# silvadirceu/acoss-1

Measured on AMD Instinct MI355X. Metric: song-pairs/sec (CSM+Qmax) on 12-d HPCP, ~2000 frames/track; MAP parity, higher is better.
Workload: dtype f32; 1 GPU; covers80-shaped synthetic HPCP (hard corpus), Serra09 CRP+Qmax, all unordered pairs; tracks=164, frames_per_track=2000, m=9, tau=1, oti=True, parallelism=pair-matrix row stripes dp1

## Files before the change

### acoss-1_amd/csrc/crp_lines.hpp

```cpp
#pragma once
#include "common.hpp"

__device__ int acoss_writelane(int value, int lane, int old) __asm("llvm.amdgcn.writelane.i32");

namespace acoss {

constexpr unsigned kNone = 0x7fffu;

__device__ __forceinline__ unsigned pk_min_u16(unsigned a, unsigned b) {
  typedef unsigned short u16x2 __attribute__((ext_vector_type(2)));
  return __builtin_bit_cast(unsigned, __builtin_elementwise_min(__builtin_bit_cast(u16x2, a), __builtin_bit_cast(u16x2, b)));
}
__device__ __forceinline__ unsigned pk_max_u16(unsigned a, unsigned b) {
  typedef unsigned short u16x2 __attribute__((ext_vector_type(2)));
  return __builtin_bit_cast(unsigned, __builtin_elementwise_max(__builtin_bit_cast(u16x2, a), __builtin_bit_cast(u16x2, b)));
}
__device__ __forceinline__ unsigned pk_add_u16(unsigned a, unsigned b) {
  typedef unsigned short u16x2 __attribute__((ext_vector_type(2)));
  return __builtin_bit_cast(unsigned, __builtin_bit_cast(u16x2, a) + __builtin_bit_cast(u16x2, b));
}
__device__ __forceinline__ unsigned pk_subsat_u16(unsigned a, unsigned b) {
  typedef unsigned short u16x2 __attribute__((ext_vector_type(2)));
  return __builtin_bit_cast(unsigned, __builtin_elementwise_sub_sat(__builtin_bit_cast(u16x2, a), __builtin_bit_cast(u16x2, b)));
}
// ... 132 lines not shown
#pragma unroll
    for (int h = 0; h < NP; ++h) ne = gather_flags(ne, (pv[h] ^ PP) + 0x7fff7fffu, h);
    return ~ne;
  }
  __device__ __forceinline__ uint32_t le8(unsigned x) const {
    const unsigned X4 = (x - base8 + 0x80u) * 0x01010101u;
    uint32_t le8 = 0;
#pragma unroll
    for (int h = 0; h < NP / 2; ++h) le8 = gather_flags8(le8, X4 - w8[h], h);
    return le8;
  }
  __device__ __forceinline__ uint32_t le16(unsigned x) const {
    const unsigned X2 = (x + 0x8000u) * 0x10001u;
    uint32_t le = 0;
#pragma unroll
    for (int h = 0; h < NP; ++h) le = gather_flags(le, X2 - pv[h], h);
    return le;
  }
  __device__ __forceinline__ void min_max_lane(unsigned* a_io, unsigned* b_io) const {
    unsigned a = *a_io, b = *b_io;
#pragma unroll
    for (int h = 0; h < NP; ++h) {
      a = pk_min_u16(a, pv[h]);
      b = pk_max_u16(b, pk_add_u16(pv[h], 0x00010001u) & 0x7fff7fffu);
    }
    *a_io = a;
    *b_io = b;
  }
  static __device__ __forceinline__ void min_max_wave(unsigned a, unsigned b, unsigned* mn, unsigned* mx) {
    a = min(a & 0xffffu, a >> 16);
    b = max(b & 0xffffu, b >> 16);
    *mn = wave_min_u32(a);
    const unsigned m = wave_max_u32(b);
    *mx = m ? m - 1 : 0u;
  }
  __device__ __forceinline__ void min_max(unsigned* mn, unsigned* mx) const {
    unsigned a = 0xffffffffu, b = 0u;
    min_max_lane(&a, &b);
    min_max_wave(a, b, mn, mx);
  }
  __device__ __forceinline__ unsigned min_greater_lane(unsigned x) const { return swar_min_greater(pv, x); }
  __device__ __forceinline__ unsigned min_greater(unsigned x) const { return wave_min_u32(min_greater_lane(x)); }
  static constexpr bool kHist = true;
  __device__ __forceinline__ bool hist_rank(unsigned hint, int rho, unsigned* hist, unsigned* P, int* le,
                                            int* less, unsigned* hbase) const {
    if constexpr (WIN) {
      *hbase = base8;
      const bool exact0 = base8 == 0u;
      hist_fill_w8(w8, hist);
      return hist_place(hist, rho, base8, 0, exact0, P, le, less);
    } else {
      const unsigned base = hint > 64u ? hint - 64u : 0u;
      *hbase = base;
      hist_clear(hist);
      const HistAddr HA(hist);
      const unsigned below = base > 0u ? cnt16(base - 1u) : 0u;
#pragma unroll
      for (int h = 0; h < NP; ++h) {
#pragma unroll
        for (int half = 0; half < 2; ++half) {
          const unsigned c = (half ? (pv[h] >> 16) : (pv[h] & 0xffffu)) - base;
          hist_add(hist, HA, c, c < 128u);
        }
      }
      return hist_place(hist, rho, base, wave_sum((int)below), true, P, le, less);
    }
  }
};

template <int KPL>
struct Line : Codes<KPL / 2, true> {
  static_assert(KPL == 32, "split word order assumes 32 elements per lane");
  static constexpr int kHalves = 1;
  __device__ __forceinline__ int ebase() const {
    int e = (threadIdx.x & 63) * KPL;
    asm volatile("" : "+v"(e));
    return e;
  }
  __device__ __forceinline__ int elem(int eb, int b) const { return eb + b; }
  static __device__ __forceinline__ int lane_of(int e) { return e / KPL; }
  static __device__ __forceinline__ int bit_of(int e) { return e % KPL; }
  __device__ __forceinline__ unsigned sample() const { return this->pv[0] & 0xffffu; }
  template <bool STORED_SPLIT>
  __device__ __forceinline__ void load_lanes(const uint16_t* col0, size_t lane_stride, int n) {
    const int lane = threadIdx.x & 63;
    const int base = lane * KPL;
    const uint16_t* src = col0 + (base < n ? (size_t)lane * lane_stride : (size_t)0);
    this->no_window();
    unsigned w[KPL / 2];
#pragma unroll
    for (int q = 0; q < KPL / 8; ++q) {
      const uint4 v = reinterpret_cast<const uint4*>(src)[q];
      w[4 * q + 0] = v.x;
      w[4 * q + 1] = v.y;
      w[4 * q + 2] = v.z;
      w[4 * q + 3] = v.w;
    }
    if (STORED_SPLIT) {
#pragma unroll
      for (int h = 0; h < KPL / 2; ++h) this->pv[h] = w[h];
    } else {
#pragma unroll
      for (int h = 0; h < KPL / 2; ++h)
        this->pv[h] = __builtin_amdgcn_perm(w[8 + (h >> 1)], w[h >> 1], (h & 1) ? 0x07060302u : 0x05040100u);
    }
    if (base >= n) {
#pragma unroll
      for (int h = 0; h < KPL / 2; ++h) this->pv[h] = kNone * 0x10001u;
    }
  }
  __device__ __forceinline__ uint32_t eq_mask(unsigned P) const {
    if (this->eq_in_win(P)) return this->eq8(P);
    return this->eq16(P);
  }
  __device__ __forceinline__ uint32_t le_mask(unsigned x) const {
    if (this->in_win(x)) return this->le8(x);
    return this->le16(x);
  }
};

template <int KQ>
struct LineS : Codes<KQ / 2, KQ == 16> {
  static_assert(KQ == 8 || KQ == 16, "short lines: 8 or 16 elements per lane");
  static constexpr bool kWin = KQ == 16;
  static constexpr int kHalves = 1;
  static constexpr uint32_t kMaskAll = ((1u << (KQ / 2)) - 1u) * 0x10001u;
  static constexpr uint32_t kWinLo = ((1u << (KQ / 4)) - 1u) * 0x10001u;
  static __device__ __forceinline__ uint32_t wmask(uint32_t m) {
    return (m & kWinLo) | ((m >> (8 - KQ / 4)) & (kWinLo << (KQ / 4)));
  }
  static __device__ __forceinline__ int q_of_bit(int b) { return b < 16 ? b : b - 16 + KQ / 2; }
  static __device__ __forceinline__ int bit_of_q(int q) { return q < KQ / 2 ? q : q - KQ / 2 + 16; }
  __device__ __forceinline__ int ebase() const {
    int e = threadIdx.x & 63;
    asm volatile("" : "+v"(e));
    return e;
  }
  __device__ __forceinline__ int elem(int eb, int b) const { return eb + 64 * q_of_bit(b); }
  static __device__ __forceinline__ int lane_of(int e) { return e & 63; }
  static __device__ __forceinline__ int bit_of(int e) { return bit_of_q(e >> 6); }
  __device__ __forceinline__ unsigned sample() const {
    const int lane = threadIdx.x & 63;
    unsigned t[KQ / 2];
#pragma unroll
    for (int k = 0; k < KQ / 2; ++k) t[k] = this->pv[k];
#pragma unroll
    for (int bit = 1, n = KQ / 2; n > 1; bit <<= 1, n >>= 1) {
      const bool sel = (lane & bit) != 0;
#pragma unroll
      for (int k = 0; k < n / 2; ++k) t[k] = sel ? t[2 * k + 1] : t[2 * k];
    }
    return (lane & (KQ / 2)) ? (t[0] >> 16) : (t[0] & 0xffffu);
  }
  template <class AT>
  __device__ __forceinline__ void load(AT addr, int n) {
    const int lane = threadIdx.x & 63;
    this->no_window();
    unsigned v[KQ];
#pragma unroll
    for (int q = 0; q < KQ; ++q) v[q] = *addr(min(lane + 64 * q, n - 1));
#pragma unroll
    for (int q = 0; q < KQ; ++q) v[q] = lane + 64 * q < n ? v[q] : kNone;
#pragma unroll
    for (int h = 0; h < KQ / 2; ++h) this->pv[h] = v[h] | (v[h + KQ / 2] << 16);
  }
  __device__ __forceinline__ uint32_t eq_mask(unsigned P) const {
    if constexpr (kWin) {
      if (this->in_win(P) && (P > this->base8 || this->base8 == 0u)) return wmask(this->eq8(P));
    }
    return this->eq16(P) & kMaskAll;
  }
  __device__ __forceinline__ uint32_t le_mask(unsigned x) const {
    if constexpr (kWin) {
      if (this->in_win(x)) return wmask(this->le8(x));
    }
    return this->le16(x);
  }
};

template <int KQ>
__device__ __forceinline__ uint32_t lane_words(uint32_t mask) {
  uint32_t out = 0;
#pragma unroll
  for (int q = 0; q < KQ; ++q) {
    const unsigned long long bal = __ballot((mask >> LineS<KQ>::bit_of_q(q)) & 1u);
    out = (uint32_t)acoss_writelane((int)(uint32_t)bal, 2 * q, (int)out);
    out = (uint32_t)acoss_writelane((int)(uint32_t)(bal >> 32), 2 * q + 1, (int)out);
  }
  return out;
}

struct Line2 {
  Line<32> A, B;
  static constexpr int kHalves = 2;
  static constexpr bool kHist = false;
  __device__ __forceinline__ int ebase() const { return A.ebase(); }
  __device__ __forceinline__ int elem(int eb, int b) const { return b < 32 ? eb + b : 2048 + eb + (b - 32); }
  static __device__ __forceinline__ int lane_of(int e) { return e < 2048 ? (e >> 5) : 64 + ((e - 2048) >> 5); }
  static __device__ __forceinline__ int bit_of(int e) { return e & 31; }
  __device__ __forceinline__ unsigned sample() const {
    const unsigned a = A.sample(), b = B.sample();
    return (threadIdx.x & 1) ? b : a;
  }
  __device__ __forceinline__ void build_window(unsigned c) {
    A.build_window(c);
    B.build_window(c);
  }
  __device__ __forceinline__ int count_le(unsigned x) const {
    if (A.in_win(x)) return wave_sum((int)(A.cnt8(x) + B.cnt8(x)));
    return wave_sum((int)(A.cnt16(x) + B.cnt16(x)));
  }
  __device__ __forceinline__ uint64_t eq_mask(unsigned P) const {
    if (A.eq_in_win(P)) return (uint64_t)A.eq8(P) | ((uint64_t)B.eq8(P) << 32);
    return (uint64_t)A.eq16(P) | ((uint64_t)B.eq16(P) << 32);
  }
  __device__ __forceinline__ uint64_t le_mask(unsigned x) const {
    if (A.in_win(x)) return (uint64_t)A.le8(x) | ((uint64_t)B.le8(x) << 32);
    return (uint64_t)A.le16(x) | ((uint64_t)B.le16(x) << 32);
  }
  __device__ __forceinline__ void min_max(unsigned* mn, unsigned* mx) const {
    unsigned a = 0xffffffffu, b = 0u;
    A.min_max_lane(&a, &b);
    B.min_max_lane(&a, &b);
    Line<32>::min_max_wave(a, b, mn, mx);
  }
  __device__ __forceinline__ unsigned min_greater(unsigned x) const {
    return wave_min_u32(min(A.min_greater_lane(x), B.min_greater_lane(x)));
  }
};

}
```

### acoss-1_amd/csrc/crp_split.hip

```cpp
#include <cstdlib>
#include <cstring>
#include <type_traits>

#include "crp_internal.hpp"
#include "crp_lines.hpp"

namespace acoss {

namespace {

constexpr int kMS = 9;


struct PairView {
  const float* X;
  const float* X2;
  const float* Yr;
  int nq, nr, tau;
  const float* NXq;
  const float* NXr;
  int Mp, Np;
};

__device__ __forceinline__ PairView pair_view(const CrpBatch& B, int p) {
// ... 177 lines not shown
      }
    }
    typedef __attribute__((address_space(1))) char gchar;
    typedef uint32_t u32x4 __attribute__((ext_vector_type(4)));
    typedef __attribute__((address_space(1))) u32x4 gu4;
    u32x4* tq = reinterpret_cast<u32x4*>(tile);
    const int cc = lane - (kMS - 1);
    if (jb + kSysCols > V.Np) {
#pragma unroll
      for (int h = 0; h < 16; ++h) hw[h] = col < V.Np ? hw[h] : kNone * 0x10001u;
    }
    if (cc >= 0) {
      uint16_t* tc = tile + cc;
#pragma unroll
      for (int h = 0; h < 16; ++h) {
        tc[h * kSysCols] = (uint16_t)hw[h];
        tc[(h + 16) * kSysCols] = (uint16_t)(hw[h] >> 16);
      }
    }
    __builtin_amdgcn_wave_barrier();
    u32x4 pr[4], pq[4];
#pragma unroll
    for (int k = 0; k < 4; ++k) pr[k] = tq[min(lane + 64 * k, kTilePieces - 1)];
#pragma unroll
    for (int k = 0; k < 4; ++k) asm volatile("" : "+v"(pr[k].x), "+v"(pr[k].y), "+v"(pr[k].z), "+v"(pr[k].w));
#pragma unroll
    for (int k = 0; k < 4; ++k) {
      const int t = lane + 64 * k;
      const int row = t / 7;
      const int c = jb + 8 * (t - 7 * row);
      if (t < kTilePieces && c < V.Np && (!PARTIAL || row < rows))
        *(gu4*)((gchar*)(gu16*)Hr + (unsigned)(row * ldr + c) * 2u) = pr[k];
    }
    __builtin_amdgcn_wave_barrier();
    if (cc >= 0) {
      const int f = (cc >> 1) & 3;
#pragma unroll
      for (int q = 0; q < 4; ++q) tq[cc * 4 + (q ^ f)] = u32x4{hw[4 * q], hw[4 * q + 1], hw[4 * q + 2], hw[4 * q + 3]};
    }
    __builtin_amdgcn_wave_barrier();
#pragma unroll
    for (int k = 0; k < 4; ++k) {
      const int t = min(lane + 64 * k, kTilePieces - 1), c = t >> 2;
      pq[k] = tq[c * 4 + ((t & 3) ^ ((c >> 1) & 3))];
    }
#pragma unroll
    for (int k = 0; k < 4; ++k) asm volatile("" : "+v"(pq[k].x), "+v"(pq[k].y), "+v"(pq[k].z), "+v"(pq[k].w));
    __builtin_amdgcn_wave_barrier();
    gu16* hcb = (gu16*)(Hc + ((size_t)strip * ldc + jb) * kSR);
#pragma unroll
    for (int k = 0; k < 4; ++k) {
      const int t = lane + 64 * k;
      if (t < kTilePieces && jb + (t >> 2) < V.Np)
        __builtin_nontemporal_store(pq[k], (gu4*)((gchar*)hcb + (unsigned)t * 16u));
    }
  }
  __syncthreads();
  const int padw = (int)((V.Np + 31) & ~31) - V.Np;
  for (int e = threadIdx.x; e < kSR * 32; e += kThreads) {
    const int r = e >> 5, c = e & 31;
    if (c < padw && r < rows) Hr[(size_t)r * ldr + V.Np + c] = (uint16_t)kNone;
  }
}

__device__ __forceinline__ int popc(uint32_t m) { return __builtin_popcount(m); }
__device__ __forceinline__ int popc(uint64_t m) { return __builtin_popcountll(m); }
__device__ __forceinline__ int ctz(uint32_t m) { return __builtin_ctz(m); }
__device__ __forceinline__ int ctz(uint64_t m) { return __builtin_ctzll(m); }

constexpr unsigned kNoHint = 0xffffffffu;

template <class LT>
__device__ __forceinline__ unsigned prefix_of_rank(const LT& L, int rho, unsigned a, unsigned b, int n,
                                                   unsigned hint, int* le_out, int* less_out, int* passes) {
  int c_b = n;
  int c_am1 = 0;
  int mode = (hint != kNoHint) ? 0 : 3;
  unsigned step = 1;
  constexpr unsigned kNext = (2u << 0) | (1u << 2) | (3u << 4) | (1u << 6) | (2u << 8) | (3u << 10) | (3u << 12) |
                             (3u << 14);
  constexpr unsigned kDouble = (1u << 3) | (1u << 4);
  while (a < b) {
    const unsigned w = b - a, mid = (a + b) >> 1;
    const unsigned th = hint < a ? a : (hint > b ? b : hint);
    const unsigned tdown = w > step ? b - step : a;
    const unsigned tup = w > step ? a + step - 1 : mid;
    const unsigned t = mode == 0 ? th : (mode == 1 ? tdown : (mode == 2 ? tup : mid));
    const int c = L.count_le(t);
    ++*passes;
    const unsigned g = (unsigned)(rho - c) >> 31;
    b = g ? t : b;
    c_b = g ? c : c_b;
    a = g ? a : t + 1;
    c_am1 = g ? c_am1 : c;
    const unsigned idx = 2u * (unsigned)mode + g;
    step <<= (kDouble >> idx) & 1u;
    mode = (int)((kNext >> (2u * idx)) & 3u);
  }
  *le_out = c_b;
  *less_out = c_am1;
  return a;
}

struct Hint {
  unsigned P;
  float dens;
};

template <class LT>
__device__ __forceinline__ unsigned sample_hint(const LT& L, int n, float kappa, unsigned* hist) {
  const int lane = threadIdx.x & 63;
  const unsigned v = L.sample();
  const bool ok = v != kNone;
  const int ns = __popcll(__ballot(ok));
  const int k = min(max((int)((float)(n - 1) * kappa * (float)ns * __builtin_amdgcn_rcpf((float)n)), 0), ns - 1);
  const unsigned lo = wave_min_u32(v), hi = wave_max_u32(ok ? v : 0u);
  if (lo >= hi) return lo > 0x7f80u ? 0x7f80u : lo;
  const unsigned range = hi - lo;
  const int sh = range < 128u ? 0 : 25 - __builtin_clz(range);
  reinterpret_cast<uint2*>(hist)[lane] = make_uint2(0u, 0u);
  __builtin_amdgcn_wave_barrier();
  if (ok) __hip_atomic_fetch_add(hist + ((v - lo) >> sh), 1u, __ATOMIC_RELAXED, __HIP_MEMORY_SCOPE_WAVEFRONT);
  __builtin_amdgcn_wave_barrier();
  const uint2 hv = reinterpret_cast<const uint2*>(hist)[lane];
  const int sl = (int)(hv.x + hv.y);
  const int S = wave_incl_scan(sl);
  const int E = S - sl;
  const int src = __builtin_ctzll(__ballot(E <= k && k < S));
  const int Es = __builtin_amdgcn_readlane(E, src);
  const int h0 = __builtin_amdgcn_readlane((int)hv.x, src);
  const unsigned bin = 2u * (unsigned)src + (k >= Es + h0 ? 1u : 0u);
  __builtin_amdgcn_wave_barrier();
  const unsigned P = lo + (bin << sh) + ((1u << sh) >> 1);
  return P > 0x7f80u ? 0x7f80u : P;
}

__device__ __forceinline__ bool hist_next(const unsigned* hist, unsigned base, unsigned P, unsigned* Pn, int* cnt) {
  const int lane = threadIdx.x & 63;
  const uint2 hv = reinterpret_cast<const uint2*>(hist)[lane];
  const unsigned b0 = base + 2u * (unsigned)lane;
  const bool n0 = hv.x != 0u && b0 > P, n1 = hv.y != 0u && b0 + 1u > P;
  const unsigned long long m = __ballot(n0 || n1);
  if (!m) return false;
  const int src = __builtin_ctzll(m);
  const unsigned x = (unsigned)__builtin_amdgcn_readlane((int)hv.x, src);
  const unsigned y = (unsigned)__builtin_amdgcn_readlane((int)hv.y, src);
  const unsigned c0 = base + 2u * (unsigned)src;
  const bool first = x != 0u && c0 > P;
  *Pn = first ? c0 : c0 + 1u;
  *cnt = (int)(first ? x : y);
  return true;
}

struct alignas(16) WaveLds {
  int list[64];
  uint32_t words[128];
  uint32_t hist[128];
  uint32_t sink[64];
  float gv[64 * kMS];
};

struct Group {
  unsigned P;
  int g;
  int elem;
  unsigned key;
  int off;
  __device__ __forceinline__ bool mine(int lane) const { return (unsigned)(lane - off) < (unsigned)g; }
};

template <class LT, class KF>
__device__ __forceinline__ Group group_keys(const LT& L, unsigned P, int g, const KF& keyf, WaveLds& W) {
  const int lane = threadIdx.x & 63;
  const int ebase = L.ebase();
  auto m = L.eq_mask(P);
  const int cnt = popc(m);
  int idx = wave_incl_scan(cnt) - cnt;
  while (m) {
    W.list[idx++] = L.elem(ebase, ctz(m));
    m &= m - 1;
  }
  __builtin_amdgcn_wave_barrier();
  const int e_me = W.list[lane < g ? lane : 0];
  const float nq_me = keyf.V.NXq[keyf.qi(e_me)], nr_me = keyf.V.NXr[keyf.rj(e_me)];
  for (int t = lane; t < kMS * g; t += 64) {
    const int k = t / kMS, u = t - k * kMS;
    const int e = W.list[k];
    W.gv[t] = cell_gram(keyf.V, (keyf.qi(e) + u) * keyf.V.tau, (keyf.rj(e) + u) * keyf.V.tau);
  }
  __builtin_amdgcn_wave_barrier();
  Group G;
  G.P = P;
  G.g = g;
  G.off = 0;
  G.elem = lane < g ? e_me : 0;
  G.key = 0xffffffffu;
  if (lane < g) {
    float dot = W.gv[lane * kMS];
#pragma unroll
    for (int u = 1; u < kMS; ++u) dot = dot + W.gv[lane * kMS + u];
    const float d2 = (nq_me - 2.0f * dot) + nr_me;
    G.key = __builtin_bit_cast(unsigned, d2 > 0.0f ? d2 : 0.0f);
  }
  __builtin_amdgcn_wave_barrier();
  return G;
}

template <class LT, class KF>
__device__ __forceinline__ void group_keys2(const LT& L, unsigned P1, int g1, unsigned P2, int g2, const KF& keyf,
                                            WaveLds& W, Group* G1, Group* G2) {
  const int lane = threadIdx.x & 63;
  const int ebase = L.ebase();
  auto m1 = L.eq_mask(P1);
  auto m2 = L.eq_mask(P2);
  const int c1 = popc(m1), c2 = popc(m2);
  const int packed = c1 | (c2 << 16);
  const int sc = wave_incl_scan(packed) - packed;
  int i1 = sc & 0xffff, i2 = g1 + (sc >> 16);
  while (m1) {
    W.list[i1++] = L.elem(ebase, ctz(m1));
    m1 &= m1 - 1;
  }
  while (m2) {
    W.list[i2++] = L.elem(ebase, ctz(m2));
    m2 &= m2 - 1;
  }
  __builtin_amdgcn_wave_barrier();
  const int g = g1 + g2;
  const int e_me = W.list[lane < g ? lane : 0];
  const float nq_me = keyf.V.NXq[keyf.qi(e_me)], nr_me = keyf.V.NXr[keyf.rj(e_me)];
  for (int t = lane; t < kMS * g; t += 64) {
    const int k = t / kMS, u = t - k * kMS;
    const int e = W.list[k];
    W.gv[t] = cell_gram(keyf.V, (keyf.qi(e) + u) * keyf.V.tau, (keyf.rj(e) + u) * keyf.V.tau);
  }
  __builtin_amdgcn_wave_barrier();
  unsigned key = 0xffffffffu;
  if (lane < g) {
    float dot = W.gv[lane * kMS];
#pragma unroll
    for (int u = 1; u < kMS; ++u) dot = dot + W.gv[lane * kMS + u];
    const float d2 = (nq_me - 2.0f * dot) + nr_me;
    key = __builtin_bit_cast(unsigned, d2 > 0.0f ? d2 : 0.0f);
  }
  __builtin_amdgcn_wave_barrier();
  const int elem = lane < g ? e_me : 0;
  *G1 = Group{P1, g1, elem, lane < g1 ? key : 0xffffffffu, 0};
  *G2 = Group{P2, g2, elem, (lane >= g1 && lane < g) ? key : 0xffffffffu, g1};
}

__device__ __forceinline__ unsigned group_min(const Group& G) {
  return wave_min_u32(G.mine(threadIdx.x & 63) ? G.key : 0xffffffffu);
}

__device__ __forceinline__ unsigned group_rank(const Group& G, int rho) {
  const int lane = threadIdx.x & 63;
  int cl = 0, ce = 0;
  for (int k = 0; k < G.g; ++k) {
    const unsigned o = (unsigned)lane_bcast((int)G.key, k);
    cl += o < G.key;
    ce += o == G.key;
  }
  const bool act = lane < G.g;
  const int src = __builtin_ctzll(__ballot(act && cl <= rho && rho < cl + ce));
  return (unsigned)lane_bcast((int)G.key, src);
}

__device__ __forceinline__ void group_rank2(const Group& G, int rho, unsigned* v0, unsigned* v1) {
  const int lane = threadIdx.x & 63;
  int cl = 0, ce = 0;
  for (int k = 0; k < G.g; ++k) {
    const unsigned o = (unsigned)lane_bcast((int)G.key, k);
    cl += o < G.key;
    ce += o == G.key;
  }
  const bool act = lane < G.g;
  const int s0 = __builtin_ctzll(__ballot(act && cl <= rho && rho < cl + ce));
  const int s1 = __builtin_ctzll(__ballot(act && cl <= rho + 1 && rho + 1 < cl + ce));
  *v0 = (unsigned)lane_bcast((int)G.key, s0);
  *v1 = (unsigned)lane_bcast((int)G.key, s1);
}

template <class LT, class F>
__device__ __forceinline__ void group_rounds(const LT& L, unsigned P, int g, WaveLds& W, F fn) {
  const int lane = threadIdx.x & 63;
  auto m = L.eq_mask(P);
  const int cnt = popc(m);
  int idx = wave_incl_scan(cnt) - cnt;
  const int ebase = L.ebase();
  for (int r0 = 0; r0 < g; r0 += 64) {
    while (m && idx < r0 + 64) {
      const int q = ctz(m);
      m &= m - 1;
      W.list[idx - r0] = L.elem(ebase, q);
      ++idx;
    }
    __builtin_amdgcn_wave_barrier();
    if (lane < min(64, g - r0)) fn(W.list[lane]);
    __builtin_amdgcn_wave_barrier();
  }
}

__device__ __forceinline__ unsigned hist_bin_of_rank(const unsigned* hist, int* rho) {
  const int lane = threadIdx.x & 63;
  const unsigned c0 = hist[4 * lane], c1 = hist[4 * lane + 1], c2 = hist[4 * lane + 2], c3 = hist[4 * lane + 3];
  const int tot = (int)(c0 + c1 + c2 + c3);
  const int ex = wave_incl_scan(tot) - tot;
  const int r = *rho;
  int bin = -1, below = ex;
  if (r >= ex && r < ex + tot) {
    if (r < below + (int)c0) {
      bin = 0;
    } else if (r < below + (int)(c0 + c1)) {
      bin = 1;
      below += c0;
    } else if (r < below + (int)(c0 + c1 + c2)) {
      bin = 2;
      below += c0 + c1;
    } else {
      bin = 3;
      below += c0 + c1 + c2;
    }
  }
  const int src = __builtin_ctzll(__ballot(bin >= 0));
  *rho = r - lane_bcast(below, src);
  return (unsigned)(4 * src + lane_bcast(bin, src));
}

template <class LT, class KF>
__device__ __forceinline__ unsigned big_group_rank(const LT& L, unsigned P, int rho, int g, const KF& keyf, WaveLds& W) {
  const int lane = threadIdx.x & 63;
  unsigned* hist = reinterpret_cast<unsigned*>(W.gv);
  unsigned hi8 = 0, lo8 = 0;
#pragma unroll 1
  for (int pass = 0; pass < 2; ++pass) {
    for (int b = lane; b < 256; b += 64) hist[b] = 0u;
    __builtin_amdgcn_wave_barrier();
    group_rounds(L, P, g, W, [&](int e) {
      const unsigned k = keyf(e);
      if (pass == 0)
        atomicAdd(&hist[(k >> 8) & 0xffu], 1u);
      else if (((k >> 8) & 0xffu) == hi8)
        atomicAdd(&hist[k & 0xffu], 1u);
    });
    __builtin_amdgcn_wave_barrier();
    const unsigned bin = hist_bin_of_rank(hist, &rho);
    __builtin_amdgcn_wave_barrier();
    if (pass == 0)
      hi8 = bin;
    else
      lo8 = bin;
  }
  return (P << 16) | (hi8 << 8) | lo8;
}

template <class LT, class KF>
__device__ __forceinline__ unsigned rank_in_prefix(const LT& L, unsigned P, int rho, int g, const KF& keyf, WaveLds& W,
                                   Group* cache) {
  if (g <= 64) {
    if (cache->g < 0 || cache->P != P) *cache = group_keys(L, P, g, keyf, W);
    return group_rank(*cache, rho);
  }
  return big_group_rank(L, P, rho, g, keyf, W);
}

struct Plan {
  unsigned Pl, hbase, Ph2;
  int le, less, gh2, lo, hi;
  float q, lo_f, hi_f;
  bool found, next_ok, both;
};

template <class LT, class KF>
__device__ __forceinline__ Plan line_plan(const LT& L, int n, float kappa, WaveLds& W, Hint* hint) {
  Plan pl;
  pl.q = (float)(n - 1) * kappa;
  pl.lo_f = floorf(pl.q);
  pl.hi_f = ceilf(pl.q);
  pl.lo = (int)pl.lo_f;
  pl.hi = (int)pl.hi_f;
  const int lo = pl.lo, hi = pl.hi;
  unsigned kmin = 0, kmax = 0x7f80u;
  const bool hinted = hint->P != kNoHint;
  if (!hinted) L.min_max(&kmin, &kmax);
  int le = 0, less = 0;
  int passes = 0;
  unsigned Pl = 0u, hbase = 0u;
  bool found = false;
  if constexpr (LT::kHist) {
    if (hinted) found = L.hist_rank(hint->P, lo, W.hist, &Pl, &le, &less, &hbase);
  }
  if (!found) Pl = prefix_of_rank(L, lo, kmin, kmax, n, hint->P, &le, &less, &passes);
  hint->P = Pl;
  hint->dens = hinted ? 0.5f * hint->dens + 0.5f * (float)(le - less) : (float)(le - less);
  pl.Pl = Pl;
  pl.hbase = hbase;
  pl.le = le;
  pl.less = less;
  pl.found = found;
  pl.Ph2 = 0u;
  pl.gh2 = 0;
  pl.next_ok = hi != lo && hi >= le && found && hist_next(W.hist, hbase, Pl, &pl.Ph2, &pl.gh2);
  pl.both = pl.next_ok && le - less <= 64 && (le - less) + pl.gh2 <= 64;
  return pl;
}

template <class LT, class KF>
__device__ __forceinline__ void line_groups(const LT& L, const Plan& pl, const KF& keyf, WaveLds& W, Group* c_lo,
                                            Group* c_hi, unsigned* vlo_o, unsigned* vhi_o) {
  const unsigned Pl = pl.Pl;
  const int le = pl.le, less = pl.less, lo = pl.lo, hi = pl.hi;
  unsigned vlo, vhi;
  if (pl.both) {
    group_keys2(L, Pl, le - less, pl.Ph2, pl.gh2, keyf, W, c_lo, c_hi);
    vlo = group_rank(*c_lo, lo - less);
    vhi = group_min(*c_hi);
  } else if (hi != lo && hi < le && le - less <= 64) {
    *c_lo = group_keys(L, Pl, le - less, keyf, W);
    group_rank2(*c_lo, lo - less, &vlo, &vhi);
  } else {
    vlo = rank_in_prefix(L, Pl, lo - less, le - less, keyf, W, c_lo);
    vhi = vlo;
  }
  if (!pl.both && hi != lo && !(hi < le && le - less <= 64)) {
    if (hi < le) {
      vhi = rank_in_prefix(L, Pl, hi - less, le - less, keyf, W, c_lo);
    } else {
      unsigned Ph;
      int gh;
      if (pl.next_ok) {
        Ph = pl.Ph2;
        gh = pl.gh2;
      } else {
        Ph = L.min_greater(Pl);
        gh = L.count_le(Ph) - le;
      }
      vhi = rank_in_prefix(L, Ph, 0, gh, keyf, W, c_hi);
    }
  }
  *vlo_o = vlo;
  *vhi_o = vhi;
}

__device__ __forceinline__ void plan_threshold(const Plan& pl, unsigned vlo, unsigned vhi, float* thr, float* T) {
  const float slo = sqrt_rn(__builtin_bit_cast(float, vlo));
  float th;
  if (pl.lo_f == pl.hi_f) {
    th = slo;
  } else {
    const float shi = sqrt_rn(__builtin_bit_cast(float, vhi));
    const float aa = slo * (pl.hi_f - pl.q);
    const float bb = shi * (pl.q - pl.lo_f);
    th = aa + bb;
  }
  *thr = th;
  *T = sq_threshold(th);
}

template <class LT, class KF>
__device__ __forceinline__ void line_threshold(const LT& L, int n, float kappa, const KF& keyf, WaveLds& W, Group* c_lo,
                               Group* c_hi, float* thr, float* T, Hint* hint) {
  const Plan pl = line_plan<LT, KF>(L, n, kappa, W, hint);
  unsigned vlo, vhi;
  line_groups(L, pl, keyf, W, c_lo, c_hi, &vlo, &vhi);
  plan_threshold(pl, vlo, vhi, thr, T);
}

template <class LT, class KF>
__device__ __forceinline__ auto le_bits(const LT& L, unsigned Tbits, const KF& keyf, WaveLds& W, const Group& c_lo,
                            const Group& c_hi) {
  const unsigned T16 = Tbits >> 16;
  const int lane = threadIdx.x & 63;
  const auto word = L.le_mask(T16);
  const bool lo_hit = c_lo.g >= 0 && c_lo.P == T16, hi_hit = c_hi.g >= 0 && c_hi.P == T16;
  W.words[lane] = 0xffffffffu;
  if (LT::kHalves == 2) W.words[64 + lane] = 0xffffffffu;
  __builtin_amdgcn_wave_barrier();
  if (lo_hit || hi_hit) {
    const bool cmine = lo_hit ? c_lo.mine(lane) : c_hi.mine(lane);
    const unsigned ckey = lo_hit ? c_lo.key : c_hi.key;
    const int celem = lo_hit ? c_lo.elem : c_hi.elem;
    if (cmine && ckey > Tbits) atomicAnd(&W.words[LT::lane_of(celem)], ~(1u << LT::bit_of(celem)));
  } else {
    const int g = wave_sum(popc(L.eq_mask(T16)));
    if (g == 0) return word;
    if (g <= 64) {
      const Group G = group_keys(L, T16, g, keyf, W);
      if (lane < G.g && G.key > Tbits) atomicAnd(&W.words[LT::lane_of(G.elem)], ~(1u << LT::bit_of(G.elem)));
    } else {
      group_rounds(L, T16, g, W, [&](int e) {
        if (keyf(e) > Tbits) atomicAnd(&W.words[LT::lane_of(e)], ~(1u << LT::bit_of(e)));
      });
    }
  }
  __builtin_amdgcn_wave_barrier();
  if constexpr (LT::kHalves == 2)
    return word & (((uint64_t)W.words[64 + lane] << 32) | W.words[lane]);
  else
    return word & W.words[lane];
}

constexpr int kRowsLds = 4 * (int)sizeof(WaveLds) + kSR * 64 * 4;
constexpr int kRowsLds2 = 4 * (int)sizeof(WaveLds) + kSR * 128 * 4;
static_assert(4 * kTileBytes <= kRowsLds, "the sweep's staging tiles must fit the row select's LDS");

template <int J>
__device__ __forceinline__ void transpose_stage(uint32_t (&a)[32]) {
  constexpr uint32_t m = J == 16 ? 0x0000ffffu : J == 8 ? 0x00ff00ffu : J == 4 ? 0x0f0f0f0fu : J == 2 ? 0x33333333u
                                                                                                      : 0x55555555u;
#pragma unroll
  for (int k = 0; k < 32; ++k) {
    if (k & J) continue;
    const uint32_t t = ((a[k] >> J) ^ a[k + J]) & m;
    a[k + J] ^= t;
    a[k] ^= t << J;
  }
}

__device__ __forceinline__ void transpose32(uint32_t (&a)[32]) {
  transpose_stage<16>(a);
  transpose_stage<8>(a);
  transpose_stage<4>(a);
  transpose_stage<2>(a);
  transpose_stage<1>(a);
}

template <int KQ>
struct LineOf {
  using T = LineS<KQ>;
};
template <>
struct LineOf<0> {
  using T = Line<32>;
};
template <>
struct LineOf<2> {
  using T = Line2;
};

template <int NW, int KQ, int RB>
__device__ __forceinline__ void rows_body(const PairView& V, int p, int strip, const uint16_t* Hr, int ldr,
                                          float kappa, float* __restrict__ thr,
                                          float* __restrict__ Tq, int64_t thr_stride, uint32_t* __restrict__ RT,
                                          int64_t rt_stride, int ld, WaveLds* wl, uint32_t (*rowbits)[RB]) {
  using LT = typename LineOf<KQ>::T;
  const int i0 = strip * kSR;
  const int w = __builtin_amdgcn_readfirstlane(threadIdx.x >> 6), lane = threadIdx.x & 63;
  WaveLds& W = wl[w];
  constexpr int RPW = kSR / NW;
  Hint hint{kNoHint, 1.0f};
  auto load_row = [&](LT& Ld, int i) {
    int64_t rowoff = (int64_t)(i - i0) * ldr;
    asm volatile("" : "+s"(rowoff));
    if constexpr (KQ == 0) {
      Ld.template load_lanes<false>(Hr + rowoff, 32, V.Np);
    } else if constexpr (KQ == 2) {
      Ld.A.template load_lanes<false>(Hr + rowoff, 32, V.Np);
      Ld.B.template load_lanes<false>(Hr + rowoff + 2048, 32, V.Np - 2048);
    } else {
      const uint16_t* row = Hr + rowoff;
      Ld.load([&](int e) { return row + (unsigned)e; }, V.Np);
    }
  };
  constexpr bool kPF = KQ != 2;
  auto row = [&](LT& L, int r, auto&& prefetch) {
    const int i = i0 + r;
    uint64_t word = 0;
    if (i < V.Mp) {
      if (hint.P == kNoHint) hint.P = sample_hint(L, V.Np, kappa, W.hist);
      if constexpr (KQ != 8) {
        if (hint.P != kNoHint) L.build_window(hint.P);
      }
      prefetch();
      const LineCells<true> keyf{V, i};
      float th, T;
      Group c_lo, c_hi;
      c_lo.g = c_hi.g = -1;
      line_threshold(L, V.Np, kappa, keyf, W, &c_lo, &c_hi, &th, &T, &hint);
      if (lane == 0) {
        thr[(size_t)p * thr_stride + i] = th;
        Tq[(size_t)p * thr_stride + i] = T;
      }
      word = le_bits(L, __builtin_bit_cast(unsigned, T), keyf, W, c_lo, c_hi);
      if constexpr (KQ == 8 || KQ == 16) word = lane_words<KQ>((uint32_t)word);
    }
    rowbits[r][lane] = (uint32_t)word;
    if constexpr (KQ == 2) rowbits[r][64 + lane] = (uint32_t)(word >> 32);
  };
  const int r1 = (w + 1) * RPW;
  {
    LT Lnext;
    if (kPF && i0 + w * RPW < V.Mp) load_row(Lnext, i0 + w * RPW);
#pragma unroll 1
    for (int r = w * RPW; r < r1; ++r) {
      LT L;
      if (i0 + r < V.Mp) {
        if constexpr (kPF)
          L = Lnext;
        else
          load_row(L, i0 + r);
      }
      row(L, r, [&] {
        if (kPF && r + 1 < r1 && i0 + r + 1 < V.Mp) load_row(Lnext, i0 + r + 1);
      });
    }
  }
  __syncthreads();
  uint32_t* out = RT + (size_t)p * rt_stride + (size_t)strip * ld;
  for (int b = threadIdx.x; 32 * b < V.Np; b += NW * 64) {
    uint32_t a[32];
#pragma unroll
    for (int r = 0; r < 32; ++r) a[r] = rowbits[r][b];
    transpose32(a);
    uint32_t* o = out + 32 * b;
    if (32 * b + 32 <= ld) {
#pragma unroll
      for (int q = 0; q < 32; q += 4) *reinterpret_cast<uint4*>(o + q) = make_uint4(a[q], a[q + 1], a[q + 2], a[q + 3]);
    } else {
#pragma unroll
      for (int q = 0; q < 32; ++q)
        if (32 * b + q < V.Np) o[q] = a[q];
    }
  }
}

template <int KQ>
constexpr int kSweepWPE = KQ == 8 ? 5 : 4;
struct SweepArgs {
  CrpBatch B;
  KeyPlanes K;
  int ldr, ldc;
  int64_t kstride;
  float kappa;
  float* thr;
  float* Tq;
  int64_t thr_stride;
  uint32_t* RT;
  int64_t rt_stride;
  int ld, short_n;
};
struct ColsArgs {
  CrpBatch B;
  KeyPlanes K;
  int ldc;
  int64_t kstride;
  float kappa;
  const uint32_t* RT;
  float* thr;
  float* Tq;
  int64_t thr_stride;
  uint32_t* maskT;
  int64_t mask_stride;
  int ld, short_n;
};
template <int KQ>
constexpr int kSweepLds = KQ == 2 ? kRowsLds2 : kRowsLds;

template <int KQ>
__device__ __forceinline__ void sweep_rows_block(const SweepArgs& A, int strip, int p, char* smem) {
  constexpr int RB = KQ == 2 ? 128 : 64;
  const CrpBatch& B = A.B;
  const KeyPlanes& K = A.K;
  const int ldr = A.ldr, ldc = A.ldc, ld = A.ld, short_n = A.short_n;
  const int64_t kstride = A.kstride, thr_stride = A.thr_stride, rt_stride = A.rt_stride;
  const float kappa = A.kappa;
  float* thr = A.thr;
  float* Tq = A.Tq;
  uint32_t* RT = A.RT;
  const PairView V = pair_view(B, p);
  const int i0 = strip * kSR;
  if (i0 >= V.Mp || V.Np <= 0) return;
  uint16_t* Hr = K.hr + (size_t)p * kstride + (size_t)i0 * ldr;
  if (i0 + kSR <= V.Mp)
    sweep_body_sys<false>(V, p, strip, K, ldr, ldc, kstride, Hr, smem);
  else
    sweep_body_sys<true>(V, p, strip, K, ldr, ldc, kstride, Hr, smem);
  __syncthreads();
  WaveLds* wl = reinterpret_cast<WaveLds*>(smem);
  uint32_t(*rowbits)[RB] = reinterpret_cast<uint32_t(*)[RB]>(smem + 4 * sizeof(WaveLds));
  if (KQ == 8 || V.Np <= short_n)
    rows_body<4, 8, RB>(V, p, strip, Hr, ldr, kappa, thr, Tq, thr_stride, RT, rt_stride, ld, wl, rowbits);
  else if (KQ == 16)
    rows_body<4, 16, RB>(V, p, strip, Hr, ldr, kappa, thr, Tq, thr_stride, RT, rt_stride, ld, wl, rowbits);
  else if (KQ == 2 && V.Np > 2048)
    rows_body<4, 2, RB>(V, p, strip, Hr, ldr, kappa, thr, Tq, thr_stride, RT, rt_stride, ld, wl, rowbits);
  else
    rows_body<4, 0, RB>(V, p, strip, Hr, ldr, kappa, thr, Tq, thr_stride, RT, rt_stride, ld, wl, rowbits);
}

template <int KQ>
__global__ __launch_bounds__(kThreads, kSweepWPE<KQ>) void k_sweep_rows9(SweepArgs A) {
  __shared__ __attribute__((aligned(16))) char smem[kSweepLds<KQ>];
  sweep_rows_block<KQ>(A, blockIdx.x, blockIdx.y, smem);
}

constexpr int kCPWLong = 2;
constexpr int kCPWShort = 4;
template <int KQ>
constexpr int kCPW = (KQ == 8 || KQ == 16) ? kCPWShort : kCPWLong;
constexpr int kColsWPE = 4;
template <int KQ>
constexpr int kColsPerBlock = 4 * kCPW<KQ>;

template <int KQ>
__device__ __forceinline__ void cols_body(const PairView& V, int p, int j0, int jend, const KeyPlanes& K, int ldc,
                                          int64_t kstride, float kappa, const uint32_t* __restrict__ RT,
                                          float* __restrict__ thr, float* __restrict__ Tq, int64_t thr_stride,
                                          uint32_t* __restrict__ maskT, int64_t mask_stride, int ld, WaveLds& W) {
  constexpr int KPL = 32;
  using LT = typename LineOf<KQ>::T;
  const int lane = threadIdx.x & 63;
  Hint hint{kNoHint, 1.0f};
  auto load_col = [&](LT& Ld, int j) {
    int64_t coloff = (int64_t)p * kstride + (int64_t)j * kSR;
    asm volatile("" : "+s"(coloff));
    if constexpr (KQ == 0) {
      Ld.template load_lanes<true>(K.hc + coloff, (size_t)ldc * kSR, V.Mp);
    } else if constexpr (KQ == 2) {
      Ld.A.template load_lanes<true>(K.hc + coloff, (size_t)ldc * kSR, V.Mp);
      Ld.B.template load_lanes<true>(K.hc + coloff + (size_t)64 * ldc * kSR, (size_t)ldc * kSR, V.Mp - 2048);
    } else {
      const uint16_t* col = K.hc + coloff;
      Ld.load([&](int e) { return col + (unsigned)((e >> 5) * ldc * kSR + (e & 15) * 2 + ((e >> 4) & 1)); }, V.Mp);
    }
  };
  auto column = [&](LT& L, int j) {
    if (hint.P == kNoHint) hint.P = sample_hint(L, V.Mp, kappa, W.hist);
    if constexpr (KQ != 8) {
      if (hint.P != kNoHint) L.build_window(hint.P);
    }
    const size_t w = (size_t)p * mask_stride + (size_t)(lane * KPL < V.Mp ? lane : 0) * ld + j;
    const uint32_t rt = RT[w];
    const size_t w2 = (size_t)p * mask_stride + (size_t)(2048 + lane * KPL < V.Mp ? 64 + lane : 0) * ld + j;
    const uint32_t rt2 = KQ == 2 ? RT[w2] : 0u;
    const LineCells<false> keyf{V, j};
    float th, Tc;
    Group c_lo, c_hi;
    c_lo.g = c_hi.g = -1;
    line_threshold(L, V.Mp, kappa, keyf, W, &c_lo, &c_hi, &th, &Tc, &hint);
    if (lane == 0) {
      thr[(size_t)p * thr_stride + j] = th;
      Tq[(size_t)p * thr_stride + j] = Tc;
    }
    uint64_t bits = le_bits(L, __builtin_bit_cast(unsigned, Tc), keyf, W, c_lo, c_hi);
    if constexpr (KQ == 8 || KQ == 16) bits = lane_words<KQ>((uint32_t)bits);
    if (lane * KPL < V.Mp) maskT[w] = (uint32_t)bits & rt;
    if (KQ == 2 && 2048 + lane * KPL < V.Mp) maskT[w2] = (uint32_t)(bits >> 32) & rt2;
  };
  constexpr bool kPF = KQ != 2;
  {
    LT Lnext;
    if (kPF && j0 < jend) load_col(Lnext, j0);
#pragma unroll 1
    for (int j = j0; j < jend; ++j) {
      LT L;
      if constexpr (kPF)
        L = Lnext;
      else
        load_col(L, j);
      if (kPF && j + 1 < jend) load_col(Lnext, j + 1);
      column(L, j);
    }
  }
}

template <int KQ>
__device__ __forceinline__ void cols_block(const ColsArgs& A, int lin, int ncb, int nblk, WaveLds* wl) {
  const CrpBatch& B = A.B;
  const KeyPlanes& K = A.K;
  const int ldc = A.ldc, ld = A.ld, short_n = A.short_n;
  const int64_t kstride = A.kstride, thr_stride = A.thr_stride, mask_stride = A.mask_stride;
  const float kappa = A.kappa;
  const uint32_t* RT = A.RT;
  float* thr = A.thr;
  float* Tq = A.Tq;
  uint32_t* maskT = A.maskT;
  const int lb = xcd_remap(lin, nblk);
  const int p = lb / ncb;
  const PairView V = pair_view(B, p);
  const int j0 = (lb - p * ncb) * kColsPerBlock<KQ> + __builtin_amdgcn_readfirstlane(threadIdx.x >> 6) * kCPW<KQ>;
  const int jend = min(j0 + kCPW<KQ>, V.Np);
  WaveLds& W = wl[__builtin_amdgcn_readfirstlane(threadIdx.x >> 6)];
  if (KQ == 8 || V.Mp <= short_n)
    cols_body<8>(V, p, j0, jend, K, ldc, kstride, kappa, RT, thr, Tq, thr_stride, maskT, mask_stride, ld, W);
  else if (KQ == 16)
    cols_body<16>(V, p, j0, jend, K, ldc, kstride, kappa, RT, thr, Tq, thr_stride, maskT, mask_stride, ld, W);
  else if (KQ == 2 && V.Mp > 2048)
    cols_body<2>(V, p, j0, jend, K, ldc, kstride, kappa, RT, thr, Tq, thr_stride, maskT, mask_stride, ld, W);
  else
    cols_body<0>(V, p, j0, jend, K, ldc, kstride, kappa, RT, thr, Tq, thr_stride, maskT, mask_stride, ld, W);
}

template <int KQ>
__global__ __launch_bounds__(256, kColsWPE) void k_sel_cols9(ColsArgs A) {
  __shared__ WaveLds wl[4];
  cols_block<KQ>(A, blockIdx.y * gridDim.x + blockIdx.x, gridDim.x, gridDim.x * gridDim.y, wl);
}

}

static int split_kq(int L, int* short_n) {
  static const bool no_short = getenv("ACOSS_NO_SHORT") != nullptr;
  *short_n = no_short ? 0 : 512;
  return L > 2048 ? 2 : (no_short ? 0 : (L <= 512 ? 8 : (L <= 1024 ? 16 : 0)));
}

static SweepArgs sweep_args(const CrpBatch& B, void* kplanes, int ldk, int64_t kstride, int nb,
                            float kappa, float* thr_r, float* T_r, int64_t thr_stride, uint32_t* RT,
                            int64_t mask_stride, int ld, int short_n) {
  const size_t plane = (size_t)nb * kstride;
  const KeyPlanes K{static_cast<uint16_t*>(kplanes), static_cast<uint16_t*>(kplanes) + plane};
  return SweepArgs{B, K, ldk, ldk, kstride, kappa, thr_r, T_r, thr_stride, RT, mask_stride, ld, short_n};
}

static ColsArgs cols_args(const CrpBatch& B, void* kplanes, int ldk, int64_t kstride, int nb, float kappa,
                          const uint32_t* RT, float* thr_c, float* T_c, int64_t thr_stride, uint32_t* maskT,
                          int64_t mask_stride, int ld, int short_n) {
  const size_t plane = (size_t)nb * kstride;
  const KeyPlanes K{static_cast<uint16_t*>(kplanes), static_cast<uint16_t*>(kplanes) + plane};
  return ColsArgs{B, K, ldk, kstride, kappa, RT, thr_c, T_c, thr_stride, maskT, mask_stride, ld, short_n};
}

int launch_crp_split(const CrpBatch& B, int nb, int L, float kappa, void* kplanes, int ldk,
                     int64_t kstride,
                     uint32_t* RT, float* thr_r, float* T_r, float* thr_c, float* T_c, int64_t thr_stride,
                     uint32_t* maskT, int64_t mask_stride, int ld, hipStream_t s) {
  if (B.m != kMS || B.tau != 1 || L > 4096) return 1;
  const int nstrips = (L + kSR - 1) / kSR;
  int short_n;
  const int kq = split_kq(L, &short_n);
  const SweepArgs SA = sweep_args(B, kplanes, ldk, kstride, nb, kappa, thr_r, T_r, thr_stride, RT, mask_stride,
                                  ld, short_n);
  const ColsArgs CA = cols_args(B, kplanes, ldk, kstride, nb, kappa, RT, thr_c, T_c, thr_stride, maskT, mask_stride,
                                ld, short_n);
  auto launch = [&](auto kqc) -> int {
    constexpr int KQ = decltype(kqc)::value;
    prof_begin(PH_SWEEP, s);
    hipLaunchKernelGGL(k_sweep_rows9<KQ>, dim3(nstrips, nb), dim3(kThreads), 0, s, SA);
    ACOSS_LAUNCH_CHECK();
    prof_end(PH_SWEEP, s);
// ... 15 lines not shown
```

Baseline: 96070 song-pairs/s.

## Defer per-row tie-group key resolution into a batched per-wave run flush

When a row's quantile falls in a small tie group, the row no longer resolves it right away. It records the group's elements in per-wave LDS and continues. After all of a wave's rows are processed, it computes the exact distance keys for every deferred element together, ranks them to get each row's threshold, and patches the row bit words with atomics. Rows whose threshold lands outside the predicted bucket are reloaded and resolved the old way. The intent is to batch the scattered exact-key recomputation and ranking across rows to improve wave utilisation. The cost is more LDS per block (possible occupancy loss) and extra fallback complexity.

```diff
diff --git a/acoss-1_amd/csrc/crp_lines.hpp b/acoss-1_amd/csrc/crp_lines.hpp
--- a/acoss-1_amd/csrc/crp_lines.hpp
+++ b/acoss-1_amd/csrc/crp_lines.hpp
@@ -308,9 +308,10 @@
     }
     return (lane & (KQ / 2)) ? (t[0] >> 16) : (t[0] & 0xffffu);
   }
-  template <class AT>
+  template <bool FRESH = false, class AT>
   __device__ __forceinline__ void load(AT addr, int n) {
-    const int lane = threadIdx.x & 63;
+    int lane = threadIdx.x & 63;
+    if (FRESH) asm volatile("" : "+v"(lane));
     this->no_window();
     unsigned v[KQ];
 #pragma unroll
diff --git a/acoss-1_amd/csrc/crp_split.hip b/acoss-1_amd/csrc/crp_split.hip
--- a/acoss-1_amd/csrc/crp_split.hip
+++ b/acoss-1_amd/csrc/crp_split.hip
@@ -353,12 +353,29 @@
   return true;
 }
 
+constexpr int kRunMax = 8;
+constexpr int kRunCap = 128;
+struct RunRec {
+  unsigned Pl, Ph;
+  int off, g1, g2;
+  int rho;
+  int two;
+  int pad;
+};
+
 struct alignas(16) WaveLds {
   int list[64];
   uint32_t words[128];
   uint32_t hist[128];
   uint32_t sink[64];
   float gv[64 * kMS];
+};
+
+struct alignas(16) RunLds {
+  int blist[kRunCap];
+  unsigned bkey[kRunCap];
+  RunRec rec[kRunMax];
+  unsigned vlo[kRunMax], vhi[kRunMax], Tl[kRunMax];
 };
 
 struct Group {
@@ -659,12 +676,26 @@
 }
 
 template <class LT, class KF>
+__device__ __forceinline__ void plan_line_threshold(const LT& L, const Plan& pl, const KF& keyf, WaveLds& W, Group* c_lo,
+                                                    Group* c_hi, float* thr, float* T) {
+  unsigned vlo, vhi;
+  line_groups(L, pl, keyf, W, c_lo, c_hi, &vlo, &vhi);
+  plan_threshold(pl, vlo, vhi, thr, T);
+}
+
+template <class LT, class KF>
 __device__ __forceinline__ void line_threshold(const LT& L, int n, float kappa, const KF& keyf, WaveLds& W, Group* c_lo,
                                Group* c_hi, float* thr, float* T, Hint* hint) {
   const Plan pl = line_plan<LT, KF>(L, n, kappa, W, hint);
-  unsigned vlo, vhi;
-  line_groups(L, pl, keyf, W, c_lo, c_hi, &vlo, &vhi);
-  plan_threshold(pl, vlo, vhi, thr, T);
+  plan_line_threshold(L, pl, keyf, W, c_lo, c_hi, thr, T);
+}
+
+__device__ __forceinline__ Plan plan_ranks(int n, float kappa) {
+  Plan pl;
+  pl.q = (float)(n - 1) * kappa;
+  pl.lo_f = floorf(pl.q);
+  pl.hi_f = ceilf(pl.q);
+  return pl;
 }
 
 template <class LT, class KF>
@@ -701,9 +732,174 @@
     return word & W.words[lane];
 }
 
-constexpr int kRowsLds = 4 * (int)sizeof(WaveLds) + kSR * 64 * 4;
-constexpr int kRowsLds2 = 4 * (int)sizeof(WaveLds) + kSR * 128 * 4;
+struct Run {
+  int ntot;
+  int maxg;
+  unsigned pend;
+};
+
+template <class LT, class KF>
+__device__ __forceinline__ bool line_defer(const LT& L, const Plan& pl, int c, const KF& keyf, RunLds& B, Run& R,
+                                           uint32_t* lew) {
+  const int lane = threadIdx.x & 63;
+  const int g1 = pl.le - pl.less;
+  const bool straddle = pl.hi != pl.lo && pl.hi >= pl.le;
+  unsigned Ph = 0u;
+  int g2 = 0;
+  if (g1 > 64) return false;
+  if (straddle) {
+    if (pl.next_ok) {
+      Ph = pl.Ph2;
+      g2 = pl.gh2;
+    } else {
+      Ph = L.min_greater(pl.Pl);
+      g2 = L.count_le(Ph) - pl.le;
+    }
+  }
+  if (g2 > 64 || R.ntot + g1 + g2 > kRunCap) return false;
+  const int ebase = L.ebase();
+  auto m1 = L.eq_mask(pl.Pl);
+  decltype(m1) m2 = 0;
+  if (g2 > 0) m2 = L.eq_mask(Ph);
+  const int c1 = popc(m1), c2 = popc(m2);
+  const int packed = c1 | (c2 << 16);
+  const int sc = wave_incl_scan(packed) - packed;
+  int i1 = R.ntot + (sc & 0xffff), i2 = R.ntot + g1 + (sc >> 16);
+  const int tag = c << 24;
+  while (m1) {
+    const int e = L.elem(ebase, ctz(m1));
+    B.blist[i1++] = keyf.qi(e) | (keyf.rj(e) << 12) | tag;
+    m1 &= m1 - 1;
+  }
+  while (m2) {
+    const int e = L.elem(ebase, ctz(m2));
+    B.blist[i2++] = keyf.qi(e) | (keyf.rj(e) << 12) | tag | (1 << 27);
+    m2 &= m2 - 1;
+  }
+  const auto word = L.le_mask(pl.Pl);
+  lew[lane] = (uint32_t)word;
+  if (LT::kHalves == 2) lew[64 + lane] = (uint32_t)((uint64_t)word >> 32);
+  if (lane == 0) B.rec[c] = RunRec{pl.Pl, Ph, R.ntot, g1, g2, pl.lo - pl.less, (pl.hi != pl.lo && !straddle) ? 1 : 0, 0};
+  R.ntot += g1 + g2;
+  R.maxg = max(R.maxg, max(g1, g2));
+  R.pend |= 1u << c;
+  return true;
+}
+
+template <int NB>
+__device__ __forceinline__ unsigned cell_key_run(const PairView& V, int i, int j) {
+  static_assert(kMS % NB == 0, "whole batches");
+  const float nq = V.NXq[i], nr = V.NXr[j];
+  const f32x4* x = reinterpret_cast<const f32x4*>(V.X + (size_t)i * 12);
+  const f32x4* y = reinterpret_cast<const f32x4*>(V.Yr + (size_t)j * 12);
+  float dot = 0.0f;
+#pragma unroll
+  for (int u0 = 0; u0 < kMS; u0 += NB) {
+    f32x4 xs[NB][3], ys[NB][3];
+#pragma unroll
+    for (int k = 0; k < NB; ++k) {
+#pragma unroll
+      for (int q = 0; q < 3; ++q) {
+        xs[k][q] = x[3 * (u0 + k) + q];
+        ys[k][q] = y[3 * (u0 + k) + q];
+      }
+    }
+#pragma unroll
+    for (int k = 0; k < NB; ++k) {
+      const float g = gram12(xs[k][0], xs[k][1], xs[k][2], ys[k][0], ys[k][1], ys[k][2]);
+      dot = (u0 + k == 0) ? g : dot + g;
+    }
+  }
+  const float d2 = (nq - 2.0f * dot) + nr;
+  return __builtin_bit_cast(unsigned, d2 > 0.0f ? d2 : 0.0f);
+}
+
+template <class LT, int NB, class RL>
+__device__ __forceinline__ void run_flush(const PairView& V, const Run& R, const Plan& pq, RunLds& B, uint32_t* lew,
+                                          int lstride, float* thr, float* Tq, RL reload) {
+  if (R.pend == 0u) return;
+  const int lane = threadIdx.x & 63;
+  __builtin_amdgcn_wave_barrier();
+#pragma unroll 1
+  for (int m0 = 0; m0 < R.ntot; m0 += 64) {
+    const int m = m0 + lane;
+    const int ent = B.blist[m < R.ntot ? m : 0];
+    B.bkey[m] = cell_key_run<NB>(V, ent & 0xfff, (ent >> 12) & 0xfff);
+  }
+  __builtin_amdgcn_wave_barrier();
+#pragma unroll 1
+  for (int m0 = 0; m0 < R.ntot; m0 += 64) {
+    const int m = m0 + lane;
+    const bool act = m < R.ntot;
+    const int ent = B.blist[act ? m : 0];
+    const unsigned key = B.bkey[act ? m : 0];
+    const int c = (ent >> 24) & 7;
+    const bool second = (ent >> 27) & 1;
+    const RunRec rc = B.rec[c];
+    const int gs = second ? rc.off + rc.g1 : rc.off, gn = second ? rc.g2 : rc.g1;
+    int cl = 0, ce = 0;
+#pragma unroll 4
+    for (int k = 0; k < R.maxg; ++k) {
+      const unsigned o = B.bkey[min(gs + k, kRunCap - 1)];
+      const bool in = k < gn;
+      cl += in && o < key;
+      ce += in && o == key;
+    }
+    if (act) {
+      if (!second) {
+        if (cl <= rc.rho && rc.rho < cl + ce) B.vlo[c] = key;
+        if (rc.two && cl <= rc.rho + 1 && rc.rho + 1 < cl + ce) B.vhi[c] = key;
+      } else if (cl == 0) {
+        B.vhi[c] = key;
+      }
+    }
+  }
+  __builtin_amdgcn_wave_barrier();
+  unsigned long long bad;
+  {
+    const bool mine = lane < kRunMax && ((R.pend >> lane) & 1u);
+    const int c = mine ? lane : __builtin_ctz(R.pend);
+    const RunRec rc = B.rec[c];
+    float th, T;
+    plan_threshold(pq, B.vlo[c], B.vhi[c], &th, &T);
+    const unsigned T16 = __builtin_bit_cast(unsigned, T) >> 16;
+    const bool ok = T16 == rc.Pl || (rc.g2 > 0 && T16 > rc.Pl && T16 <= rc.Ph);
+    if (mine) {
+      thr[lane] = th;
+      Tq[lane] = T;
+      B.Tl[lane] = __builtin_bit_cast(unsigned, T);
+    }
+    bad = __ballot(mine && !ok);
+  }
+  __builtin_amdgcn_wave_barrier();
+#pragma unroll 1
+  for (int m0 = 0; m0 < R.ntot; m0 += 64) {
+    const int m = m0 + lane;
+    const bool act = m < R.ntot;
+    const int ent = B.blist[act ? m : 0];
+    const unsigned key = B.bkey[act ? m : 0];
+    const int c = (ent >> 24) & 7;
+    const bool second = (ent >> 27) & 1;
+    const unsigned Tb = B.Tl[c];
+    const int e = (ent >> 12) & 0xfff;
+    uint32_t* word = lew + c * lstride + LT::lane_of(e);
+    const uint32_t bit = 1u << LT::bit_of(e);
+    if (act && !second && key > Tb) atomicAnd(word, ~bit);
+    if (act && second && key <= Tb) atomicOr(word, bit);
+  }
+  __builtin_amdgcn_wave_barrier();
+  while (bad) {
+    const int c = __builtin_ctzll(bad);
+    bad &= bad - 1;
+    reload(c, (unsigned)__builtin_amdgcn_readfirstlane((int)B.Tl[c]));
+  }
+  __builtin_amdgcn_wave_barrier();
+}
+
+constexpr int kRowsLds = 4 * (int)(sizeof(WaveLds) + sizeof(RunLds)) + kSR * 64 * 4;
+constexpr int kRowsLds2 = 4 * (int)(sizeof(WaveLds) + sizeof(RunLds)) + kSR * 128 * 4;
 static_assert(4 * kTileBytes <= kRowsLds, "the sweep's staging tiles must fit the row select's LDS");
+static_assert(5 * kRowsLds <= 160 * 1024 && 4 * kRowsLds2 <= 160 * 1024, "sweep blocks per CU by LDS");
 
 template <int J>
 __device__ __forceinline__ void transpose_stage(uint32_t (&a)[32]) {
@@ -739,18 +935,19 @@
   using T = Line2;
 };
 
-template <int NW, int KQ, int RB>
+template <int NW, int KQ, int RB, int NB>
 __device__ __forceinline__ void rows_body(const PairView& V, int p, int strip, const uint16_t* Hr, int ldr,
                                           float kappa, float* __restrict__ thr,
                                           float* __restrict__ Tq, int64_t thr_stride, uint32_t* __restrict__ RT,
-                                          int64_t rt_stride, int ld, WaveLds* wl, uint32_t (*rowbits)[RB]) {
+                                          int64_t rt_stride, int ld, WaveLds* wl, RunLds* rl, uint32_t (*rowbits)[RB]) {
   using LT = typename LineOf<KQ>::T;
   const int i0 = strip * kSR;
   const int w = __builtin_amdgcn_readfirstlane(threadIdx.x >> 6), lane = threadIdx.x & 63;
   WaveLds& W = wl[w];
+  RunLds& B = rl[w];
   constexpr int RPW = kSR / NW;
   Hint hint{kNoHint, 1.0f};
-  auto load_row = [&](LT& Ld, int i) {
+  auto load_row = [&](LT& Ld, int i, auto fresh) {
     int64_t rowoff = (int64_t)(i - i0) * ldr;
     asm volatile("" : "+s"(rowoff));
     if constexpr (KQ == 0) {
@@ -760,10 +957,13 @@
       Ld.B.template load_lanes<false>(Hr + rowoff + 2048, 32, V.Np - 2048);
     } else {
       const uint16_t* row = Hr + rowoff;
-      Ld.load([&](int e) { return row + (unsigned)e; }, V.Np);
+      Ld.template load<decltype(fresh)::value>([&](int e) { return row + (unsigned)e; }, V.Np);
     }
   };
   constexpr bool kPF = KQ != 2;
+  static_assert(RPW <= kRunMax, "a wave's rows are one run");
+  const int r0 = w * RPW, r1 = (w + 1) * RPW;
+  Run R{0, 0, 0u};
   auto row = [&](LT& L, int r, auto&& prefetch) {
     const int i = i0 + r;
     uint64_t word = 0;
@@ -774,24 +974,24 @@
       }
       prefetch();
       const LineCells<true> keyf{V, i};
+      const Plan pl = line_plan<LT, LineCells<true>>(L, V.Np, kappa, W, &hint);
+      if (line_defer(L, pl, r - r0, keyf, B, R, &rowbits[r][0])) return;
       float th, T;
       Group c_lo, c_hi;
       c_lo.g = c_hi.g = -1;
-      line_threshold(L, V.Np, kappa, keyf, W, &c_lo, &c_hi, &th, &T, &hint);
+      plan_line_threshold(L, pl, keyf, W, &c_lo, &c_hi, &th, &T);
       if (lane == 0) {
         thr[(size_t)p * thr_stride + i] = th;
         Tq[(size_t)p * thr_stride + i] = T;
       }
       word = le_bits(L, __builtin_bit_cast(unsigned, T), keyf, W, c_lo, c_hi);
-      if constexpr (KQ == 8 || KQ == 16) word = lane_words<KQ>((uint32_t)word);
     }
     rowbits[r][lane] = (uint32_t)word;
     if constexpr (KQ == 2) rowbits[r][64 + lane] = (uint32_t)(word >> 32);
   };
-  const int r1 = (w + 1) * RPW;
   {
     LT Lnext;
-    if (kPF && i0 + w * RPW < V.Mp) load_row(Lnext, i0 + w * RPW);
+    if (kPF && i0 + w * RPW < V.Mp) load_row(Lnext, i0 + w * RPW, std::false_type{});
 #pragma unroll 1
     for (int r = w * RPW; r < r1; ++r) {
       LT L;
@@ -799,11 +999,32 @@
         if constexpr (kPF)
           L = Lnext;
         else
-          load_row(L, i0 + r);
+          load_row(L, i0 + r, std::false_type{});
       }
       row(L, r, [&] {
-        if (kPF && r + 1 < r1 && i0 + r + 1 < V.Mp) load_row(Lnext, i0 + r + 1);
+        if (kPF && r + 1 < r1 && i0 + r + 1 < V.Mp) load_row(Lnext, i0 + r + 1, std::false_type{});
       });
+    }
+  }
+  {
+    float kap = kappa;
+    asm volatile("" : "+s"(kap));
+    const Plan pq = plan_ranks(V.Np, kap);
+    float* thr0 = thr + (size_t)p * thr_stride + i0 + r0;
+    float* Tq0 = Tq + (size_t)p * thr_stride + i0 + r0;
+    run_flush<LT, NB>(V, R, pq, B, &rowbits[r0][0], RB, thr0, Tq0, [&](int c, unsigned Tbits) {
+      LT L;
+      load_row(L, i0 + r0 + c, std::true_type{});
+      const LineCells<true> keyf{V, i0 + r0 + c};
+      Group c_lo, c_hi;
+      c_lo.g = c_hi.g = -1;
+      const uint64_t word = le_bits(L, Tbits, keyf, W, c_lo, c_hi);
+      rowbits[r0 + c][lane] = (uint32_t)word;
+      if constexpr (KQ == 2) rowbits[r0 + c][64 + lane] = (uint32_t)(word >> 32);
+    });
+    if constexpr (KQ == 8 || KQ == 16) {
+#pragma unroll 1
+      for (int r = r0; r < r1; ++r) rowbits[r][lane] = lane_words<KQ>(rowbits[r][lane]);
     }
   }
   __syncthreads();
@@ -860,6 +1081,7 @@
 template <int KQ>
 __device__ __forceinline__ void sweep_rows_block(const SweepArgs& A, int strip, int p, char* smem) {
   constexpr int RB = KQ == 2 ? 128 : 64;
+  constexpr int NB = KQ == 8 ? 1 : 3;
   const CrpBatch& B = A.B;
   const KeyPlanes& K = A.K;
   const int ldr = A.ldr, ldc = A.ldc, ld = A.ld, short_n = A.short_n;
@@ -878,15 +1100,16 @@
     sweep_body_sys<true>(V, p, strip, K, ldr, ldc, kstride, Hr, smem);
   __syncthreads();
   WaveLds* wl = reinterpret_cast<WaveLds*>(smem);
-  uint32_t(*rowbits)[RB] = reinterpret_cast<uint32_t(*)[RB]>(smem + 4 * sizeof(WaveLds));
+  RunLds* rl = reinterpret_cast<RunLds*>(smem + 4 * sizeof(WaveLds));
+  uint32_t(*rowbits)[RB] = reinterpret_cast<uint32_t(*)[RB]>(smem + 4 * (sizeof(WaveLds) + sizeof(RunLds)));
   if (KQ == 8 || V.Np <= short_n)
-    rows_body<4, 8, RB>(V, p, strip, Hr, ldr, kappa, thr, Tq, thr_stride, RT, rt_stride, ld, wl, rowbits);
+    rows_body<4, 8, RB, NB>(V, p, strip, Hr, ldr, kappa, thr, Tq, thr_stride, RT, rt_stride, ld, wl, rl, rowbits);
   else if (KQ == 16)
-    rows_body<4, 16, RB>(V, p, strip, Hr, ldr, kappa, thr, Tq, thr_stride, RT, rt_stride, ld, wl, rowbits);
+    rows_body<4, 16, RB, NB>(V, p, strip, Hr, ldr, kappa, thr, Tq, thr_stride, RT, rt_stride, ld, wl, rl, rowbits);
   else if (KQ == 2 && V.Np > 2048)
-    rows_body<4, 2, RB>(V, p, strip, Hr, ldr, kappa, thr, Tq, thr_stride, RT, rt_stride, ld, wl, rowbits);
+    rows_body<4, 2, RB, NB>(V, p, strip, Hr, ldr, kappa, thr, Tq, thr_stride, RT, rt_stride, ld, wl, rl, rowbits);
   else
-    rows_body<4, 0, RB>(V, p, strip, Hr, ldr, kappa, thr, Tq, thr_stride, RT, rt_stride, ld, wl, rowbits);
+    rows_body<4, 0, RB, NB>(V, p, strip, Hr, ldr, kappa, thr, Tq, thr_stride, RT, rt_stride, ld, wl, rl, rowbits);
 }
 
 template <int KQ>
```

Result: faster. 97600 song-pairs/s, median of 6 (+1.6%).
